# bryanlimy/tf2-cyclegan

Hardware: AMD Instinct MI355X
Metric: images/sec (whole node) horse2zebra 256×256 (higher is better)
Workload: dtype bf16; 1 GPU; model=cyclegan-resnet9-patchgan, global_batch=4, per_gpu_batch=4, image_size=256, parallelism=dp1

## Files before the change

### cyclegan_amd/ops/_hip/bind.cpp

```cpp
#include <torch/extension.h>

namespace cyg {
at::Tensor conv2d_fwd(at::Tensor, at::Tensor, c10::optional<at::Tensor>,
                      int64_t, int64_t, int64_t, int64_t, int64_t, bool,
                      int64_t, double);
at::Tensor convt2d_fwd(at::Tensor, at::Tensor, c10::optional<at::Tensor>,
                       int64_t, int64_t, int64_t, int64_t, int64_t, int64_t,
                       double);
std::vector<at::Tensor> conv2d_fwd_stats(at::Tensor, at::Tensor,
                                         c10::optional<at::Tensor>, int64_t,
                                         int64_t, int64_t, int64_t, int64_t,
                                         bool, int64_t, double);
std::vector<at::Tensor> convt2d_fwd_stats(at::Tensor, at::Tensor,
                                          c10::optional<at::Tensor>, int64_t,
                                          int64_t, int64_t, int64_t, int64_t,
                                          int64_t, double);
at::Tensor conv2d_dgrad(at::Tensor, at::Tensor, int64_t, int64_t, int64_t,
                        int64_t, int64_t, int64_t, int64_t, bool);
at::Tensor convt2d_dgrad(at::Tensor, at::Tensor, int64_t, int64_t, int64_t,
                         int64_t, int64_t);
at::Tensor conv2d_wgrad(at::Tensor, at::Tensor, int64_t, int64_t, int64_t,
                        int64_t, int64_t, bool);
at::Tensor mfma_probe(at::Tensor, at::Tensor);
at::Tensor mx_probe(at::Tensor, at::Tensor, int64_t, int64_t);
at::Tensor mx_probe16(at::Tensor, at::Tensor, int64_t, int64_t);
at::Tensor glds_probe(at::Tensor, at::Tensor);
at::Tensor tr_probe(int64_t);
at::Tensor quant_fp8(at::Tensor, at::Tensor);
at::Tensor quant_fp8_d(at::Tensor, at::Tensor, at::Tensor);
void amax_roll(at::Tensor, int64_t);
at::Tensor conv2d_fp8_fwd(at::Tensor, at::Tensor, at::Tensor,
                          c10::optional<at::Tensor>, c10::optional<at::Tensor>,
                          int64_t, int64_t, int64_t, int64_t, int64_t, bool, int64_t, double);
std::vector<at::Tensor> conv2d_fp8_fwd_stats(
    at::Tensor, at::Tensor, at::Tensor, c10::optional<at::Tensor>,
    c10::optional<at::Tensor>, int64_t, int64_t, int64_t, int64_t, int64_t,
    bool, int64_t, double);
std::vector<at::Tensor> instnorm_fwd(at::Tensor, at::Tensor, at::Tensor,
                                     double, int64_t, double,
                                     c10::optional<at::Tensor>,
                                     c10::optional<at::Tensor>,
                                     c10::optional<at::Tensor>, int64_t);
std::vector<at::Tensor> instnorm_fwd_q8(at::Tensor, at::Tensor, at::Tensor,
                                        double, int64_t, double,
                                        c10::optional<at::Tensor>,
                                        c10::optional<at::Tensor>,
                                        c10::optional<at::Tensor>, int64_t,
                                        at::Tensor, at::Tensor);
std::vector<at::Tensor> instnorm_bwd(at::Tensor, at::Tensor, at::Tensor,
                                     at::Tensor, at::Tensor,
                                     c10::optional<at::Tensor>, int64_t,
                                     double, c10::optional<at::Tensor>);
at::Tensor act_bwd(at::Tensor, at::Tensor, int64_t, double);
at::Tensor channel_sum(at::Tensor);
at::Tensor reflect_pad_fwd(at::Tensor, int64_t, int64_t, int64_t, int64_t);
at::Tensor reflect_pad_bwd(at::Tensor, int64_t, int64_t, int64_t, int64_t);
at::Tensor persample_loss_fwd(at::Tensor, at::Tensor, bool);
at::Tensor persample_loss_const_fwd(at::Tensor, double, bool);
std::vector<at::Tensor> persample_loss_bwd(at::Tensor, at::Tensor, at::Tensor,
                                           bool, bool, bool);
at::Tensor persample_loss_const_bwd(at::Tensor, double, at::Tensor, bool);
void adam_step_dev(at::Tensor, at::Tensor, at::Tensor, at::Tensor, at::Tensor,
                   double, double, double);
void shadow_gather(at::Tensor, at::Tensor, at::Tensor);
void adam_step(at::Tensor, at::Tensor, at::Tensor, at::Tensor, double, double,
               double, double, int64_t);
at::Tensor augment_batch(at::Tensor, at::Tensor, at::Tensor, int64_t, int64_t,
                         at::Tensor);
}

PYBIND11_MODULE(TORCH_EXTENSION_NAME, m) {
  m.def("conv2d_fwd", &cyg::conv2d_fwd);
  m.def("convt2d_fwd", &cyg::convt2d_fwd);
  m.def("conv2d_fwd_stats", &cyg::conv2d_fwd_stats);
  m.def("convt2d_fwd_stats", &cyg::convt2d_fwd_stats);
  m.def("conv2d_dgrad", &cyg::conv2d_dgrad);
  m.def("convt2d_dgrad", &cyg::convt2d_dgrad);
  m.def("conv2d_wgrad", &cyg::conv2d_wgrad);
  m.def("mfma_probe", &cyg::mfma_probe);
  m.def("mx_probe", &cyg::mx_probe);
  m.def("mx_probe16", &cyg::mx_probe16);
  m.def("glds_probe", &cyg::glds_probe);
  m.def("tr_probe", &cyg::tr_probe);
  m.def("quant_fp8", &cyg::quant_fp8);
  m.def("quant_fp8_d", &cyg::quant_fp8_d);
  m.def("amax_roll", &cyg::amax_roll);
  m.def("conv2d_fp8_fwd", &cyg::conv2d_fp8_fwd);
  m.def("conv2d_fp8_fwd_stats", &cyg::conv2d_fp8_fwd_stats);
  m.def("instnorm_fwd", &cyg::instnorm_fwd, py::arg("x"), py::arg("gamma"),
        py::arg("beta"), py::arg("eps"), py::arg("act"), py::arg("slope"),
        py::arg("residual"), py::arg("psum") = py::none(),
        py::arg("psq") = py::none(), py::arg("nslabs") = 0);
  m.def("instnorm_fwd_q8", &cyg::instnorm_fwd_q8, py::arg("x"),
        py::arg("gamma"), py::arg("beta"), py::arg("eps"), py::arg("act"),
        py::arg("slope"), py::arg("residual"), py::arg("psum"),
        py::arg("psq"), py::arg("nslabs"), py::arg("amax_prev"),
        py::arg("amax_cur"));
  m.def("instnorm_bwd", &cyg::instnorm_bwd, py::arg("dy"), py::arg("x"),
        py::arg("gamma"), py::arg("mean"), py::arg("rstd"), py::arg("yact"),
        py::arg("act"), py::arg("slope"), py::arg("beta") = py::none());
  m.def("act_bwd", &cyg::act_bwd);
  m.def("channel_sum", &cyg::channel_sum);
  m.def("reflect_pad_fwd", &cyg::reflect_pad_fwd);
  m.def("reflect_pad_bwd", &cyg::reflect_pad_bwd);
  m.def("persample_loss_fwd", &cyg::persample_loss_fwd);
  m.def("persample_loss_const_fwd", &cyg::persample_loss_const_fwd);
  m.def("persample_loss_bwd", &cyg::persample_loss_bwd);
  m.def("persample_loss_const_bwd", &cyg::persample_loss_const_bwd);
  m.def("adam_step", &cyg::adam_step);
  m.def("adam_step_dev", &cyg::adam_step_dev);
  m.def("shadow_gather", &cyg::shadow_gather);
  m.def("augment_batch", &cyg::augment_batch);
}
```

### cyclegan_amd/ops/_hip/conv.hip

```cpp

#include <torch/extension.h>
#include <ATen/cuda/CUDAContext.h>

#include "common.h"

namespace cyg {

constexpr int BM = 128, BN = 64, BK = 64;
constexpr int NTHREADS = 256;
constexpr int LDK = BK + 8;

struct ConvParams {
  const short* __restrict__ x;
  const short* __restrict__ w;
  const short* __restrict__ bias;
  short* __restrict__ y;
  int B, H, W, Cin, OH, OW, Cout, KH, KW;
  int stride, pt, pl;
  int reflect;
  int act;  float slope;
  const float* dq;
  const float* dqb;
  long M, KTOT;
  int mtiles, ntiles;
// ... 1397 lines not shown
  if (k >= KTOT || n >= Cout) return;
  long stride = (long)ktiles * ntiles * wbn * WG_BK;
  long off = (((long)kt * ntiles + nt) * wbn + nl) * WG_BK + kl;
  float s0 = 0, s1 = 0, s2 = 0, s3 = 0;
  int sl = 0;
  for (; sl + 4 <= slices; sl += 4) {
    s0 += ws[off + (sl + 0) * stride];
    s1 += ws[off + (sl + 1) * stride];
    s2 += ws[off + (sl + 2) * stride];
    s3 += ws[off + (sl + 3) * stride];
  }
  for (; sl < slices; ++sl) s0 += ws[off + sl * stride];
  dw[(long)n * KTOT + k] = (s0 + s1) + (s2 + s3);
}

__global__ void reflect_fold_kernel(const short* __restrict__ dxp,
                                    short* __restrict__ dx,
                                    int B, int H, int W, int C,
                                    int pt, int pb, int pl, int pr) {
  long idx = (long)blockIdx.x * blockDim.x + threadIdx.x;
  int gpr = C / 8;
  long total = (long)B * H * W * gpr;
  if (idx >= total) return;
  int g = (int)(idx % gpr);
  long t = idx / gpr;
  int j = (int)(t % W);
  t /= W;
  int i = (int)(t % H);
  int b = (int)(t / H);
  int HP = H + pt + pb, WP = W + pl + pr;
// ... 421 lines not shown
                              hipStream_t stream) {
  constexpr size_t SMB = sizeof(WgSmemT<WBN>);
  if constexpr (WBN == 128) {
    static bool init = []() {
      hipFuncSetAttribute((const void*)(wgrad_glds_kernel<128>),
                          hipFuncAttributeMaxDynamicSharedMemorySize,
                          (int)SMB);
      return true;
    }();
    (void)init;
  }
  hipLaunchKernelGGL((wgrad_glds_kernel<WBN>), grid, dim3(NW * 64), SMB,
                     stream, p);
}

at::Tensor conv2d_wgrad(at::Tensor x, at::Tensor dy, int64_t KH, int64_t KW,
                        int64_t stride, int64_t pt, int64_t pl, bool reflect) {
  TORCH_CHECK(x.is_cuda() && dy.is_cuda() && x.is_contiguous() && dy.is_contiguous());
  TORCH_CHECK(x.scalar_type() == at::kBFloat16 && dy.scalar_type() == at::kBFloat16);
  TORCH_CHECK(dy.size(0) == x.size(0));
  WgradParams p{};
  p.x = (const short*)x.const_data_ptr();
  p.dy = (const short*)dy.const_data_ptr();
  p.B = x.size(0); p.H = x.size(1); p.W = x.size(2); p.Cin = x.size(3);
  p.OH = dy.size(1); p.OW = dy.size(2); p.Cout = dy.size(3);
  p.KH = KH; p.KW = KW; p.stride = stride; p.pt = pt; p.pl = pl;
  p.reflect = reflect ? 1 : 0;
  p.M = (long)p.B * p.OH * p.OW;
  p.KTOT = (long)KH * KW * p.Cin;
  const bool glds_ok = (p.Cin % 8) == 0 && (p.Cout % 8) == 0 &&
                       (long)p.B * p.H * p.W * p.Cin * 2 < (1L << 31) &&
                       p.M * p.Cout * 2 < (1L << 31);
  const int wbn = glds_ok ? conv_ntile(p.Cout) : WG_BN;
  p.ktiles = cdiv(p.KTOT, WG_BK);
  p.ntiles = cdiv(p.Cout, wbn);
  const WgSplit split = wgrad_split(p.M, p.ktiles, p.ntiles);
  p.slices = split.slices;
  p.mchunks_per_slice = split.mchunks_per_slice;
  dim3 grid((long)p.ktiles * p.ntiles * p.slices);
  auto stream = at::cuda::getCurrentCUDAStream();
  if (!glds_ok) {
    auto dw = at::zeros({p.Cout, (long)KH, (long)KW, p.Cin},
                        x.options().dtype(at::kFloat));
    p.dw = (float*)dw.mutable_data_ptr();
    hipLaunchKernelGGL(wgrad_kernel, grid, dim3(NTHREADS), 0, stream, p);
    return dw;
  }
  auto dw = at::empty({p.Cout, (long)KH, (long)KW, p.Cin},
                      x.options().dtype(at::kFloat));
  p.dw = (float*)dw.mutable_data_ptr();
  auto ws = at::empty({(long)p.slices * p.ktiles * p.ntiles * wbn * WG_BK},
                      x.options().dtype(at::kFloat));
  p.ws = (float*)ws.mutable_data_ptr();
  switch (wbn) {
    case 16: launch_wgrad_glds<16>(p, grid, stream); break;
    case 128: launch_wgrad_glds<128>(p, grid, stream); break;
    default: launch_wgrad_glds<64>(p, grid, stream);
  }
  long total = (long)p.ktiles * WG_BK * p.ntiles * wbn;
  hipLaunchKernelGGL(wgrad_reduce_kernel, dim3(cdiv(total, 256)),
                     dim3(256), 0, stream,
                     (const float*)ws.const_data_ptr(), p.dw, p.KTOT,
                     p.Cout, p.ktiles, p.ntiles, p.slices, wbn);
  return dw;
}

at::Tensor quant_fp8(at::Tensor x, at::Tensor scale) {
  TORCH_CHECK(x.is_cuda() && x.scalar_type() == at::kBFloat16 && x.is_contiguous());
  TORCH_CHECK(scale.scalar_type() == at::kFloat);
  auto y = at::empty_like(x, x.options().dtype(at::kByte));
  long n = x.numel();
  long blocks = (n / 8 + 255) / 256 + 1;
  hipLaunchKernelGGL(quant_fp8_kernel, dim3((unsigned)blocks), dim3(256), 0,
                     at::cuda::getCurrentCUDAStream(),
                     (const short*)x.const_data_ptr(),
                     (const float*)scale.const_data_ptr(),
                     (unsigned char*)y.mutable_data_ptr(), n);
  return y;
}
// ... 91 lines not shown
```

### cyclegan_amd/ops/_hip/norm_elem.hip

```cpp

#include <torch/extension.h>
#include <ATen/cuda/CUDAContext.h>

#include "common.h"

namespace cyg {

constexpr int NT = 256;

static inline int cdiv64(long a, long b) { return (int)((a + b - 1) / b); }

__global__ __launch_bounds__(NT) void in_reduce_kernel(
    const short* __restrict__ x, float* __restrict__ psum,
    float* __restrict__ psq, int B, long HW, int C, int S) {
  int b = blockIdx.x / S;
  int sl = blockIdx.x % S;
  long rows = (HW + S - 1) / S;
  long r0 = sl * rows, r1 = min(r0 + rows, HW);
  const int gpr = C / 8;
  const int tid = threadIdx.x;
  const short* xb = x + (long)b * HW * C;

  int g = tid % gpr;
  int rstep = NT / gpr;
// ... 175 lines not shown
constexpr int MASK_NONE = 0, MASK_YACT = 1, MASK_X = 2;
DEV float actbw(float d, float yy, int act, float slope) {
  if (act == ACT_RELU) return yy > 0.f ? d : 0.f;
  if (act == ACT_LRELU) return yy > 0.f ? d : d * slope;
  if (act == ACT_TANH) return d * (1.f - yy * yy);
  return d;
}

template <int MM>
__global__ __launch_bounds__(NT) void in_bwd_reduce_kernel(
    const short* __restrict__ dy, const short* __restrict__ x,
    const short* __restrict__ yact, const float* __restrict__ gamma,
    const float* __restrict__ beta, const float* __restrict__ mean,
    const float* __restrict__ rstd,
    float* __restrict__ p1, float* __restrict__ p2, int B, long HW, int C,
    int S, int act, float slope, float* __restrict__ dgb) {
  int b = blockIdx.x / S;
  int sl = blockIdx.x % S;
  if (blockIdx.x == 0)
    for (int i = threadIdx.x; i < 2 * C; i += NT) dgb[i] = 0.f;
  long rows = (HW + S - 1) / S;
  long r0 = sl * rows, r1 = min(r0 + rows, HW);
  const int gpr = C / 8;
  const int tid = threadIdx.x;
  const long base = (long)b * HW * C;

  int g = tid % gpr;
  int rstep = NT / gpr;
  int rof = tid / gpr;
  float a1[8] = {}, a2[8] = {};
  float mv[8], rv[8], gv[8] = {}, bv[8] = {};
  #pragma unroll
  for (int j = 0; j < 8; ++j) {
    mv[j] = mean[(long)b * C + g * 8 + j];
    rv[j] = rstd[(long)b * C + g * 8 + j];
// ... 153 lines not shown
        float xh = (xf - smean[c]) * rs;
        float d = b2f(dv[j]);
        if (MM == MASK_YACT) d = actbw(d, b2f(yv[j]), act, slope);
        if (MM == MASK_X)
          d = actbw(d, in_affine(xf, smean[c], rs, gamma[c], beta[c]), act,
                    slope);
        out[j] = f2b(gamma[c] * rs * (d - sm1[c] - xh * sm2[c]));
      }
      *(v8s*)(dx + off) = out;
    }
  }
}

__global__ __launch_bounds__(NT) void channel_sum_kernel(
    const short* __restrict__ x, float* __restrict__ out, long rows, int C,
    int S) {
  int sl = blockIdx.x;
  long per = (rows + S - 1) / S;
  long r0 = sl * per, r1 = min(r0 + per, rows);
  const int gpr = C / 8;
  const int tid = threadIdx.x;
  int g = tid % gpr;
  int rstep = NT / gpr;
  int rof = tid / gpr;
  float a[8] = {};
  for (long r = r0 + rof; r < r1; r += rstep) {
    v8s v = *(const v8s*)(x + r * C + g * 8);
    #pragma unroll
    for (int j = 0; j < 8; ++j) a[j] += b2f(v[j]);
  }
  __shared__ float red[NT * 17];
  #pragma unroll
  for (int j = 0; j < 8; ++j) red[tid * 17 + j] = a[j];
  __syncthreads();
  for (int c = tid; c < C; c += NT) {
    int g2 = c / 8, j = c % 8;
    float t = 0;
    for (int k = 0; k < rstep; ++k) t += red[(g2 + k * gpr) * 17 + j];
    atomicAdd(&out[c], t);
  }
}

__global__ void act_bwd_kernel(const short* __restrict__ dy,
                               const short* __restrict__ y,
                               short* __restrict__ out, long n, int act,
                               float slope) {
  long i = ((long)blockIdx.x * blockDim.x + threadIdx.x) * 8;
  if (i >= n) return;
  if (i + 8 <= n) {
    v8s dv = *(const v8s*)(dy + i);
// ... 305 lines not shown
      hipLaunchKernelGGL(kern<MASK_X>, grid, dim3(NT), 0, stream,           \
                         __VA_ARGS__);                                      \
    else if ((mm) == MASK_YACT)                                             \
      hipLaunchKernelGGL(kern<MASK_YACT>, grid, dim3(NT), 0, stream,        \
                         __VA_ARGS__);                                      \
    else                                                                    \
      hipLaunchKernelGGL(kern<MASK_NONE>, grid, dim3(NT), 0, stream,        \
                         __VA_ARGS__);                                      \
  } while (0)

std::vector<at::Tensor> instnorm_bwd(at::Tensor dy, at::Tensor x,
                                     at::Tensor gamma, at::Tensor mean,
                                     at::Tensor rstd,
                                     c10::optional<at::Tensor> yact,
                                     int64_t act, double slope,
                                     c10::optional<at::Tensor> beta) {
  TORCH_CHECK(dy.is_cuda() && dy.scalar_type() == at::kBFloat16 &&
              dy.is_contiguous() && x.is_contiguous());
  TORCH_CHECK(act == ACT_NONE || yact.has_value() ||
              ((act == ACT_RELU || act == ACT_LRELU) && beta.has_value()),
              "instnorm_bwd: act ", act, " needs yact (or beta for relu/lrelu)");
  TORCH_CHECK(!beta.has_value() ||
              (beta->scalar_type() == at::kFloat && beta->numel() == x.size(3)),
              "instnorm_bwd: beta must be fp32 [C]");
  const float* betap =
      beta.has_value() ? (const float*)beta->const_data_ptr() : nullptr;
  const int mm = act == ACT_NONE ? MASK_NONE
                                 : (yact.has_value() ? MASK_YACT : MASK_X);
  int B = x.size(0), C = x.size(3);
  long HW = (long)x.size(1) * x.size(2);
  TORCH_CHECK(C % 8 == 0 && (C / 8) <= 256 && 256 % std::min(C / 8, 256) == 0,
              "instnorm_bwd: unsupported channel count ", C);
  auto stream = at::cuda::getCurrentCUDAStream();
  auto fopt = x.options().dtype(at::kFloat);
  int S = slices_for(HW, B);
  auto dx = at::empty_like(x);
  auto dgb = at::empty({2, C}, fopt);
  auto dbeta = dgb[0];
  auto dgamma = dgb[1];
  const short* yp = yact.has_value()
                        ? (const short*)yact->const_data_ptr() : nullptr;

  auto p1 = at::empty({S, B, C}, fopt);
  auto p2 = at::empty({S, B, C}, fopt);
  LAUNCH_MM(in_bwd_reduce_kernel, mm, dim3(B * S), stream,
                     (const short*)dy.const_data_ptr(),
                     (const short*)x.const_data_ptr(), yp,
                     (const float*)gamma.const_data_ptr(), betap,
                     (const float*)mean.const_data_ptr(),
                     (const float*)rstd.const_data_ptr(),
                     (float*)p1.mutable_data_ptr(),
                     (float*)p2.mutable_data_ptr(), B, HW, C, S, (int)act,
                     (float)slope, (float*)dgb.mutable_data_ptr());
  LAUNCH_MM(in_bwd_dx_kernel, mm, dim3(B * S), stream,
                     (const short*)dy.const_data_ptr(),
                     (const short*)x.const_data_ptr(), yp,
                     (const float*)gamma.const_data_ptr(), betap,
                     (const float*)mean.const_data_ptr(),
                     (const float*)rstd.const_data_ptr(),
                     (const float*)p1.const_data_ptr(),
                     (const float*)p2.const_data_ptr(),
                     (short*)dx.mutable_data_ptr(),
                     (float*)dbeta.mutable_data_ptr(),
                     (float*)dgamma.mutable_data_ptr(), B, HW, C, S,
                     (int)act, (float)slope);
  return {dx, dgamma, dbeta};
}

at::Tensor channel_sum(at::Tensor x) {
  TORCH_CHECK(x.is_cuda() && x.scalar_type() == at::kBFloat16 && x.is_contiguous());
  int C = x.size(-1);
  long rows = x.numel() / C;
  TORCH_CHECK(C % 8 == 0 && (C / 8) <= NT && NT % (C / 8) == 0,
              "channel_sum: unsupported C ", C);
  auto out = at::empty({C}, x.options().dtype(at::kFloat));
  CHECK_HIP(hipMemsetAsync(out.mutable_data_ptr(), 0, C * sizeof(float),
                           at::cuda::getCurrentCUDAStream()));
  int S = (int)std::min<long>(512, std::max<long>(1, rows / 64));
  hipLaunchKernelGGL(channel_sum_kernel, dim3(S), dim3(NT), 0,
                     at::cuda::getCurrentCUDAStream(),
                     (const short*)x.const_data_ptr(),
                     (float*)out.mutable_data_ptr(), rows, C, S);
  return out;
}

at::Tensor act_bwd(at::Tensor dy, at::Tensor y, int64_t act, double slope) {
  TORCH_CHECK(dy.is_cuda() && dy.scalar_type() == at::kBFloat16);
  auto out = at::empty_like(dy);
  long n = dy.numel();
  long blocks = (n / 8 + 255) / 256 + 1;
  hipLaunchKernelGGL(act_bwd_kernel, dim3((unsigned)blocks), dim3(256), 0,
                     at::cuda::getCurrentCUDAStream(),
                     (const short*)dy.const_data_ptr(),
                     (const short*)y.const_data_ptr(),
                     (short*)out.mutable_data_ptr(), n, (int)act,
                     (float)slope);
  return out;
// ... 154 lines not shown
```

### cyclegan_amd/ops/conv.py

```python

from __future__ import annotations

import os
from typing import NamedTuple, Optional, Tuple

import torch
import torch.nn.functional as F

from . import backend
from .shadow import (compute_weight, compute_weight_t, compute_weight_p,
                     compute_weight_tp, compute_bias_p, compute_weight_packp,
                     compute_bias_packb, fp8_weight_shadow)

ACT_NONE, ACT_RELU, ACT_LRELU, ACT_TANH = 0, 1, 2, 3

_ACT = {None: ACT_NONE, "none": ACT_NONE, "relu": ACT_RELU, "lrelu": ACT_LRELU, "tanh": ACT_TANH}


def same_pads(in_h: int, in_w: int, kh: int, kw: int, stride: int) -> Tuple[int, int, int, int]:
    out_h = -(-in_h // stride)
    out_w = -(-in_w // stride)
    ph = max(0, (out_h - 1) * stride + kh - in_h)
    pw = max(0, (out_w - 1) * stride + kw - in_w)
    return ph // 2, ph - ph // 2, pw // 2, pw - pw // 2
# ... 65 lines not shown
    @staticmethod
    def forward(ctx, x, w, bias, stride, pads, reflect, act, slope):
        ext = backend.ext()
        cout = w.shape[0]
        xp = _pad_channels(x).contiguous()
        wc = compute_weight_p(w, x)
        bc = compute_bias_p(bias, x) if bias is not None else None
        slabs = ()
        if _want_stats(bias, act) and cout >= 8:
            y, *slabs = ext.conv2d_fwd_stats(xp, wc, bc, stride, *pads,
                                             reflect, act, slope)
        else:
            y = ext.conv2d_fwd(xp, wc, bc, stride, *pads, reflect, act, slope)
        if cout < 8:
            y = y[..., :cout].contiguous()
        ctx.save_for_backward(xp, w, y)
        ctx.conf = (stride, pads, reflect, act, slope, bias is not None,
                    x.shape[3])
        if slabs:
            ctx.set_materialize_grads(False)
            ctx.mark_non_differentiable(*slabs)
            return (y, *slabs)
        return y

    @staticmethod
    def backward(ctx, dy, *_):
        if dy is None:
            return (None,) * 8
        xp, w, y = ctx.saved_tensors
        stride, pads, reflect, act, slope, has_bias, cin = ctx.conf
        cout = w.shape[0]
        pt, pb, pl, pr = pads
        ext = backend.ext()
        dy = dy.contiguous()
        if act != ACT_NONE:
            dy = ext.act_bwd(dy, y, act, slope)
        dyp = _pad_channels(dy).contiguous()
        db = None
        if has_bias and ctx.needs_input_grad[2]:
            db = ext.channel_sum(dyp)[: dy.shape[-1]]
        dx = dw = None
        if ctx.needs_input_grad[0]:
            wt = compute_weight_tp(w, xp)
            dx = ext.conv2d_dgrad(dyp, wt, xp.shape[1], xp.shape[2], stride,
                                  pt, pb, pl, pr, reflect)
            if cin < 8:
                dx = dx[..., :cin].contiguous()
        if ctx.needs_input_grad[1]:
            dw = ext.conv2d_wgrad(xp, dyp, w.shape[1], w.shape[2], stride,
                                  pt, pl, reflect)
            if cout < 8 or cin < 8:
                dw = dw[:cout, :, :, :cin].contiguous()
            if dw.dtype != w.dtype:
                dw = dw.to(w.dtype)
        return dx, dw, db, None, None, None, None, None


def _head_packable(x, w, stride, pads, reflect) -> bool:
    import os
    if os.environ.get("CYG_NO_PACKHEAD") == "1":
        return False
    return (reflect and stride == 1 and pads == (3, 3, 3, 3)
            and w.shape[0] <= 8 and w.shape[1] == 7 and w.shape[2] == 7
            and w.shape[3] % 8 == 0 and w.shape[3] >= 8
            and x.shape[2] % 8 == 0 and x.shape[1] >= 7 and x.shape[2] >= 16)


def _fold_packed_dw(dwp: torch.Tensor, wshape) -> torch.Tensor:
    O, KH, KW, I = wshape
    d6 = dwp.view(8, 8, KH, 2, 8, I)
# ... 9 lines not shown
class _ConvHeadPackedFn(torch.autograd.Function):

    @staticmethod
    def forward(ctx, x, w, bias, act, slope):
        ext = backend.ext()
        B, H, W, Cin = x.shape
        cout = w.shape[0]
        wpk = compute_weight_packp(w, x)
        bpk = compute_bias_packb(bias, x) if bias is not None else None
        xp = ext.reflect_pad_fwd(x.contiguous(), 3, 3, 3, 5)
        xf = xp.view(B, H + 6, (W + 8) // 8, 8 * Cin)
        yp = ext.conv2d_fwd(xf, wpk, bpk, 1, 0, 0, 0, 0, False, act, slope)
        y = yp.view(B, H, W, 8)
        if cout < 8:
            y = y[..., :cout].contiguous()
        ctx.save_for_backward(xp, w, y)
        ctx.conf = (act, slope, bias is not None, cout, Cin, H, W)
        return y

    @staticmethod
    def backward(ctx, dy):
        xp, w, y = ctx.saved_tensors
        act, slope, has_bias, cout, Cin, H, W = ctx.conf
        ext = backend.ext()
        dy = dy.contiguous()
        if act != ACT_NONE:
            dy = ext.act_bwd(dy, y, act, slope)
        dyp = _pad_channels(dy).contiguous()
        db = None
        if has_bias and ctx.needs_input_grad[2]:
            db = ext.channel_sum(dyp)[: dy.shape[-1]]
        dx = dw = None
        B = dyp.shape[0]
        if ctx.needs_input_grad[0]:
            wt = compute_weight_tp(w, xp)
            dx = ext.conv2d_dgrad(dyp, wt, H, W, 1, 3, 3, 3, 3, True)
        if ctx.needs_input_grad[1]:
            xf = xp.view(B, H + 6, (W + 8) // 8, 8 * Cin)
            dy_pk = dyp.view(B, H, W // 8, 64)
            dwp = ext.conv2d_wgrad(xf, dy_pk, 7, 2, 1, 0, 0, False)
            dw = _fold_packed_dw(dwp, tuple(w.shape))
            if dw.dtype != w.dtype:
                dw = dw.to(w.dtype)
        return dx, dw, db, None, None


_FP8_MODE = False


def set_fp8_mode(on: bool):
    global _FP8_MODE
    _FP8_MODE = bool(on)


def fp8_mode() -> bool:
    return _FP8_MODE


# ... 53 lines not shown
        if fresh:
            prev.copy_(xp.detach().abs().amax().float().clamp(min=1e-12))
            twin = None
        xq = twin if twin is not None else ext.quant_fp8_d(xp, prev, cur)
        bc = compute_bias_p(bias, x) if bias is not None else None
        slabs = ()
        if (_want_stats(bias, act) and cout >= 8
                and not _knob_off("CYG_NO_FP8_STATS")):
            y, *slabs = ext.conv2d_fp8_fwd_stats(xq, wq, prev, sw, bc, stride,
                                                 *pads, reflect, act, slope)
        else:
            y = ext.conv2d_fp8_fwd(xq, wq, prev, sw, bc, stride, *pads,
                                   reflect, act, slope)
        if cout < 8:
            y = y[..., :cout].contiguous()
        ctx.save_for_backward(xp, w, y)
        ctx.conf = (stride, pads, reflect, act, slope, bias is not None,
                    x.shape[3])
        if slabs:
            ctx.set_materialize_grads(False)
            ctx.mark_non_differentiable(*slabs)
            return (y, *slabs)
        return y

    @staticmethod
    def backward(ctx, dy, *_):
        return _ConvFn.backward(ctx, dy) + (None,)


class _ConvTFn(torch.autograd.Function):
    @staticmethod
# ... 11 lines not shown
        ctx.save_for_backward(x, w, y)
        ctx.conf = (stride, pt, pl, act, slope, bias is not None)
        if slabs:
            ctx.set_materialize_grads(False)
            ctx.mark_non_differentiable(*slabs)
            return (y, *slabs)
        return y

    @staticmethod
    def backward(ctx, dy, *_):
        if dy is None:
            return (None,) * 10
        x, w, y = ctx.saved_tensors
        stride, pt, pl, act, slope, has_bias = ctx.conf
        ext = backend.ext()
        dy = dy.contiguous()
        if act != ACT_NONE:
            dy = ext.act_bwd(dy, y, act, slope)
        dx = dw = db = None
        if ctx.needs_input_grad[0]:
            wt = compute_weight_t(w, x)
            dx = ext.convt2d_dgrad(dy, wt, x.shape[1], x.shape[2], stride, pt, pl)
        if ctx.needs_input_grad[1]:
            dwc = ext.conv2d_wgrad(dy, x, w.shape[1], w.shape[2], stride,
                                   pt, pl, False)
            dw = dwc.permute(3, 1, 2, 0).contiguous()
            if dw.dtype != w.dtype:
                dw = dw.to(w.dtype)
        if has_bias and ctx.needs_input_grad[2]:
            db = dy.float().sum(dim=(0, 1, 2))
        return dx, dw, db, None, None, None, None, None, None, None


def conv2d(
    x: torch.Tensor,
    w: torch.Tensor,
    bias: Optional[torch.Tensor] = None,
    stride: int = 1,
    padding: str | Tuple[int, int, int, int] = "valid",
    pad_mode: str = "zeros",
    act: Optional[str] = None,
    slope: float = 0.2,
) -> torch.Tensor:
# ... 43 lines not shown
```

### cyclegan_amd/ops/norm.py

```python

from __future__ import annotations

import os
from typing import Optional

import torch

from . import backend
from . import conv as _conv
from .conv import (ACT_NONE, ACT_RELU, ACT_LRELU, FP8_TWIN_ATTR,
                   IN_SLABS_ATTR, _ACT, Fp8Consumer)

EPS_DEFAULT = 1e-3


def _in_ref(x, gamma, beta, eps, act, slope, residual):
    cdt = torch.float32 if x.dtype == torch.bfloat16 else x.dtype
    xf = x.to(cdt)
    mean = xf.mean(dim=(1, 2), keepdim=True)
    var = xf.var(dim=(1, 2), unbiased=False, keepdim=True)
    y = (xf - mean) * torch.rsqrt(var + eps)
    y = y * gamma.to(cdt) + beta.to(cdt)
    y = y.to(x.dtype)
    if residual is not None:
# ... 33 lines not shown
        ctx.conf = (eps, act, slope, residual is not None)
        if yq is not None:
            ctx.set_materialize_grads(False)
            ctx.mark_non_differentiable(yq)
            return y, yq
        return y

    @staticmethod
    def backward(ctx, dy, *_):
        if dy is None:
            return (None,) * 11
        x, gamma, mean, rstd, y, betaf = ctx.saved_tensors
        eps, act, slope, has_res = ctx.conf
        ext = backend.ext()
        dy = dy.contiguous()
        if has_res and act != ACT_NONE:
            dy = ext.act_bwd(dy, y, act, slope)
            dres = dy
            dx, dgamma, dbeta = ext.instnorm_bwd(dy, x, gamma.float(), mean,
                                                 rstd, None, ACT_NONE, 0.0)
        else:
            dres = dy if has_res else None
            yact = y if (act != ACT_NONE and not _mask_from_x(act)) else None
            dx, dgamma, dbeta = ext.instnorm_bwd(
                dy, x, gamma.float(), mean, rstd, yact, act, slope, betaf)
        return (dx, dgamma.to(gamma.dtype), dbeta, None, None, None, dres,
                None, None, None, None)


def _slabs_for(x: torch.Tensor):
    st = getattr(x, IN_SLABS_ATTR, None)
    if st is None or x.dim() != 4:
        return None, None
    psum, psq = st
    want = (x.shape[0], x.shape[3])
    if (psum.dim() != 3 or tuple(psum.shape[1:]) != want
            or psq.shape != psum.shape or psum.device != x.device):
        return None, None
    return psum, psq


# ... 32 lines not shown
```

### cyclegan_amd/parallel/flat.py

```python

from __future__ import annotations

from typing import List

import torch


class FlatParamGroup:
    def __init__(self, module: torch.nn.Module):
        params: List[torch.nn.Parameter] = [p for p in module.parameters() if p.requires_grad]
        assert all(p.dtype == torch.float32 for p in params), "master params must be fp32"
        n = sum(p.numel() for p in params)
        dev = params[0].device
        self.flat_param = torch.empty(n, dtype=torch.float32, device=dev)
        self.flat_grad = torch.zeros(n, dtype=torch.float32, device=dev)
        self.params = params
        self._offsets = []
        off = 0
        with torch.no_grad():
            for p in params:
                k = p.numel()
                self.flat_param[off:off + k].copy_(p.detach().reshape(-1))
                p.data = self.flat_param[off:off + k].view(p.shape)
                self._offsets.append((off, k))
                off += k
        self.attach_grads()

    def attach_grads(self):
        for p, (off, k) in zip(self.params, self._offsets):
            p.grad = self.flat_grad[off:off + k].view(p.shape)

    def bump_versions(self):
        for p in self.params:
            torch.autograd.graph.increment_version(p)

    def set_grads(self, grads):
        torch._foreach_copy_(
            [p.grad for p in self.params],
            [g.reshape(p.shape) for p, g in zip(self.params, grads)])

    def zero_grad(self):
        self.flat_grad.zero_()
        self.attach_grads()

    def check_views(self) -> bool:
        pp = self.flat_param.data_ptr()
        gp = self.flat_grad.data_ptr()
        ok = True
        for p in self.params:
            ok &= p.data.data_ptr() >= pp and p.data.data_ptr() < pp + self.flat_param.numel() * 4
            ok &= p.grad is not None and gp <= p.grad.data_ptr() < gp + self.flat_grad.numel() * 4
        return ok
```

### cyclegan_amd/trainer.py

```python

from __future__ import annotations

import os
from typing import Dict, Optional

import torch

from .models import Generator, Discriminator
from .ops import MAE, MSE, MSE_const, backend
from .ops.adam import FusedAdam
from .parallel import DistContext, GradSync, FlatParamGroup


class CycleGAN:
    LAMBDA_CYCLE = 10.0
    LAMBDA_IDENTITY = 0.5 * 10.0

    def __init__(self, args, ctx: DistContext):
        self.ctx = ctx
        self.device = ctx.device
        self.global_batch_size = args.global_batch_size
        self.compute_dtype = getattr(args, "compute_dtype", None) or (
            torch.bfloat16 if self.device.type == "cuda" else torch.float32)
        self._fp8 = bool(getattr(args, "fp8", False))
# ... 109 lines not shown
            "loss_F/loss": F_loss, "loss_F/cycle": F_cycle_loss,
            "loss_F/identity": F_identity_loss,
            "loss_F/total": F_loss + F_cycle_loss + F_identity_loss,
            "loss_X/loss": self.discriminator_loss(self.X(x),
                                                   discriminate_fake_x),
            "loss_Y/loss": self.discriminator_loss(self.Y(y),
                                                   discriminate_fake_y),
        }

    _GROUP_LOSS = (("G", "loss_G/total"), ("F", "loss_F/total"),
                   ("X", "loss_X/loss"), ("Y", "loss_Y/loss"))

    def _grads_for(self, losses: Dict[str, torch.Tensor], name: str,
                   retain: bool):
        key = dict(self._GROUP_LOSS)[name]
        self.groups[name].set_grads(
            torch.autograd.grad(losses[key], self.groups[name].params,
                                retain_graph=retain))

    def _optimize(self):
        for opt in self.optimizers.values():
            opt.step()
        for g in self.groups.values():
            g.bump_versions()
        self._refresh_shadows()
        if getattr(self, "_fp8", False):
            from .ops import fp8_state
            fp8_state.roll()

    def train_step(self, x, y) -> Dict[str, torch.Tensor]:
        x, y = self._cast(x), self._cast(y)
        if x.shape[0] == 0:
            return self._empty_train_step()
# ... 237 lines not shown
```

Baseline: 340.2 images/s.

## Write weight and norm gradients directly into flat gradient buffers via grad sink

Adds a grad-sink mechanism so conv wgrad, transposed-conv wgrad, packed-7x7 fold, instnorm bwd and bias channel_sum write (or accumulate) fp32 gradients straight into the flat parameter gradient views, instead of returning temporaries that are permuted, cast and then copied with foreach_copy. It also skips weight-gradient computation for frozen leaf parameters that are not in the current group, so each autograd.grad call only computes wgrad for its own group. This cuts extra kernels, allocations and copies in backward. The cost is global state coupling autograd functions to the trainer, and accumulate paths that rely on touched flags.

```diff
diff --git a/cyclegan_amd/ops/_hip/bind.cpp b/cyclegan_amd/ops/_hip/bind.cpp
--- a/cyclegan_amd/ops/_hip/bind.cpp
+++ b/cyclegan_amd/ops/_hip/bind.cpp
@@ -21,6 +21,9 @@
                          int64_t, int64_t);
 at::Tensor conv2d_wgrad(at::Tensor, at::Tensor, int64_t, int64_t, int64_t,
                         int64_t, int64_t, bool);
+void conv2d_wgrad_into(at::Tensor, at::Tensor, int64_t, int64_t, int64_t,
+                       int64_t, int64_t, bool, at::Tensor, bool, bool);
+void fold_packed_dw_into(at::Tensor, at::Tensor, bool);
 at::Tensor mfma_probe(at::Tensor, at::Tensor);
 at::Tensor mx_probe(at::Tensor, at::Tensor, int64_t, int64_t);
 at::Tensor mx_probe16(at::Tensor, at::Tensor, int64_t, int64_t);
@@ -50,9 +53,11 @@
 std::vector<at::Tensor> instnorm_bwd(at::Tensor, at::Tensor, at::Tensor,
                                      at::Tensor, at::Tensor,
                                      c10::optional<at::Tensor>, int64_t,
-                                     double, c10::optional<at::Tensor>);
+                                     double, c10::optional<at::Tensor>,
+                                     c10::optional<at::Tensor>,
+                                     c10::optional<at::Tensor>, bool);
 at::Tensor act_bwd(at::Tensor, at::Tensor, int64_t, double);
-at::Tensor channel_sum(at::Tensor);
+at::Tensor channel_sum(at::Tensor, c10::optional<at::Tensor>, bool);
 at::Tensor reflect_pad_fwd(at::Tensor, int64_t, int64_t, int64_t, int64_t);
 at::Tensor reflect_pad_bwd(at::Tensor, int64_t, int64_t, int64_t, int64_t);
 at::Tensor persample_loss_fwd(at::Tensor, at::Tensor, bool);
@@ -77,6 +82,12 @@
   m.def("conv2d_dgrad", &cyg::conv2d_dgrad);
   m.def("convt2d_dgrad", &cyg::convt2d_dgrad);
   m.def("conv2d_wgrad", &cyg::conv2d_wgrad);
+  m.def("conv2d_wgrad_into", &cyg::conv2d_wgrad_into, py::arg("x"),
+        py::arg("dy"), py::arg("kh"), py::arg("kw"), py::arg("stride"),
+        py::arg("pt"), py::arg("pl"), py::arg("reflect"), py::arg("out"),
+        py::arg("accumulate"), py::arg("transpose_oi") = false);
+  m.def("fold_packed_dw_into", &cyg::fold_packed_dw_into, py::arg("dwp"),
+        py::arg("out"), py::arg("accumulate"));
   m.def("mfma_probe", &cyg::mfma_probe);
   m.def("mx_probe", &cyg::mx_probe);
   m.def("mx_probe16", &cyg::mx_probe16);
@@ -98,9 +109,12 @@
         py::arg("amax_cur"));
   m.def("instnorm_bwd", &cyg::instnorm_bwd, py::arg("dy"), py::arg("x"),
         py::arg("gamma"), py::arg("mean"), py::arg("rstd"), py::arg("yact"),
-        py::arg("act"), py::arg("slope"), py::arg("beta") = py::none());
+        py::arg("act"), py::arg("slope"), py::arg("beta") = py::none(),
+        py::arg("dgamma_out") = py::none(), py::arg("dbeta_out") = py::none(),
+        py::arg("accumulate") = false);
   m.def("act_bwd", &cyg::act_bwd);
-  m.def("channel_sum", &cyg::channel_sum);
+  m.def("channel_sum", &cyg::channel_sum, py::arg("x"),
+        py::arg("out") = py::none(), py::arg("accumulate") = false);
   m.def("reflect_pad_fwd", &cyg::reflect_pad_fwd);
   m.def("reflect_pad_bwd", &cyg::reflect_pad_bwd);
   m.def("persample_loss_fwd", &cyg::persample_loss_fwd);
diff --git a/cyclegan_amd/ops/_hip/conv.hip b/cyclegan_amd/ops/_hip/conv.hip
--- a/cyclegan_amd/ops/_hip/conv.hip
+++ b/cyclegan_amd/ops/_hip/conv.hip
@@ -1435,6 +1435,66 @@
   dw[(long)n * KTOT + k] = (s0 + s1) + (s2 + s3);
 }
 
+__global__ void wgrad_reduce_into_kernel(const float* __restrict__ ws,
+                                         float* __restrict__ out, long KTOT,
+                                         int Cout, int ktiles, int ntiles,
+                                         int slices, int wbn, int cin_g,
+                                         int taps, int co_true, int ci_true,
+                                         int tr, int accum) {
+  long idx = (long)blockIdx.x * blockDim.x + threadIdx.x;
+  long total = (long)ktiles * WG_BK * ntiles * wbn;
+  if (idx >= total) return;
+  int kl = (int)(idx % WG_BK);
+  long t = idx / WG_BK;
+  int kt = (int)(t % ktiles);
+  t /= ktiles;
+  int nl = (int)(t % wbn);
+  int nt = (int)(t / wbn);
+  long k = (long)kt * WG_BK + kl;
+  int n = nt * wbn + nl;
+  if (k >= KTOT || n >= Cout) return;
+  int tap = (int)(k / cin_g);
+  int ci = (int)(k - (long)tap * cin_g);
+  if (n >= co_true || ci >= ci_true) return;
+  long stride = (long)ktiles * ntiles * wbn * WG_BK;
+  long off = (((long)kt * ntiles + nt) * wbn + nl) * WG_BK + kl;
+  float s0 = 0, s1 = 0, s2 = 0, s3 = 0;
+  int sl = 0;
+  for (; sl + 4 <= slices; sl += 4) {
+    s0 += ws[off + (sl + 0) * stride];
+    s1 += ws[off + (sl + 1) * stride];
+    s2 += ws[off + (sl + 2) * stride];
+    s3 += ws[off + (sl + 3) * stride];
+  }
+  for (; sl < slices; ++sl) s0 += ws[off + sl * stride];
+  float s = (s0 + s1) + (s2 + s3);
+  long o = tr ? ((long)ci * taps + tap) * co_true + n
+              : ((long)n * taps + tap) * ci_true + ci;
+  out[o] = accum ? out[o] + s : s;
+}
+
+__global__ void fold_packed_dw_kernel(const float* __restrict__ dwp,
+                                      float* __restrict__ out, int O, int KH,
+                                      int KW, int I, int accum) {
+  long idx = (long)blockIdx.x * blockDim.x + threadIdx.x;
+  long total = (long)O * KH * KW * I;
+  if (idx >= total) return;
+  int ci = (int)(idx % I);
+  long t = idx / I;
+  int tx = (int)(t % KW);
+  t /= KW;
+  int ty = (int)(t % KH);
+  int co = (int)(t / KH);
+  float s = 0.f;
+  #pragma unroll
+  for (int d = 0; d < 8; ++d) {
+    int a = tx + d;
+    s += dwp[((((long)(d * 8 + co) * KH + ty) * 2 + (a >> 3)) * 8 + (a & 7)) *
+                 I + ci];
+  }
+  out[idx] = accum ? out[idx] + s : s;
+}
+
 __global__ void reflect_fold_kernel(const short* __restrict__ dxp,
                                     short* __restrict__ dx,
                                     int B, int H, int W, int C,
@@ -1886,8 +1946,10 @@
                      stream, p);
 }
 
-at::Tensor conv2d_wgrad(at::Tensor x, at::Tensor dy, int64_t KH, int64_t KW,
-                        int64_t stride, int64_t pt, int64_t pl, bool reflect) {
+static at::Tensor wgrad_impl(at::Tensor x, at::Tensor dy, int64_t KH,
+                             int64_t KW, int64_t stride, int64_t pt,
+                             int64_t pl, bool reflect, const at::Tensor* into,
+                             bool accumulate, bool transpose_oi) {
   TORCH_CHECK(x.is_cuda() && dy.is_cuda() && x.is_contiguous() && dy.is_contiguous());
   TORCH_CHECK(x.scalar_type() == at::kBFloat16 && dy.scalar_type() == at::kBFloat16);
   TORCH_CHECK(dy.size(0) == x.size(0));
@@ -1916,11 +1978,18 @@
                         x.options().dtype(at::kFloat));
     p.dw = (float*)dw.mutable_data_ptr();
     hipLaunchKernelGGL(wgrad_kernel, grid, dim3(NTHREADS), 0, stream, p);
-    return dw;
-  }
-  auto dw = at::empty({p.Cout, (long)KH, (long)KW, p.Cin},
-                      x.options().dtype(at::kFloat));
-  p.dw = (float*)dw.mutable_data_ptr();
+    if (!into) return dw;
+    auto v = transpose_oi ? dw.permute({3, 1, 2, 0}) : dw;
+    v = v.narrow(0, 0, into->size(0)).narrow(3, 0, into->size(3));
+    if (accumulate) into->add_(v); else into->copy_(v);
+    return *into;
+  }
+  at::Tensor dw;
+  if (!into) {
+    dw = at::empty({p.Cout, (long)KH, (long)KW, p.Cin},
+                   x.options().dtype(at::kFloat));
+    p.dw = (float*)dw.mutable_data_ptr();
+  }
   auto ws = at::empty({(long)p.slices * p.ktiles * p.ntiles * wbn * WG_BK},
                       x.options().dtype(at::kFloat));
   p.ws = (float*)ws.mutable_data_ptr();
@@ -1930,11 +1999,67 @@
     default: launch_wgrad_glds<64>(p, grid, stream);
   }
   long total = (long)p.ktiles * WG_BK * p.ntiles * wbn;
-  hipLaunchKernelGGL(wgrad_reduce_kernel, dim3(cdiv(total, 256)),
+  if (!into) {
+    hipLaunchKernelGGL(wgrad_reduce_kernel, dim3(cdiv(total, 256)),
+                       dim3(256), 0, stream,
+                       (const float*)ws.const_data_ptr(), p.dw, p.KTOT,
+                       p.Cout, p.ktiles, p.ntiles, p.slices, wbn);
+    return dw;
+  }
+  const int co_true = (int)into->size(transpose_oi ? 3 : 0);
+  const int ci_true = (int)into->size(transpose_oi ? 0 : 3);
+  hipLaunchKernelGGL(wgrad_reduce_into_kernel, dim3(cdiv(total, 256)),
                      dim3(256), 0, stream,
-                     (const float*)ws.const_data_ptr(), p.dw, p.KTOT,
-                     p.Cout, p.ktiles, p.ntiles, p.slices, wbn);
-  return dw;
+                     (const float*)ws.const_data_ptr(),
+                     (float*)into->mutable_data_ptr(), p.KTOT, p.Cout,
+                     p.ktiles, p.ntiles, p.slices, wbn, p.Cin, (int)(KH * KW),
+                     co_true, ci_true, transpose_oi ? 1 : 0,
+                     accumulate ? 1 : 0);
+  return *into;
+}
+
+at::Tensor conv2d_wgrad(at::Tensor x, at::Tensor dy, int64_t KH, int64_t KW,
+                        int64_t stride, int64_t pt, int64_t pl, bool reflect) {
+  return wgrad_impl(x, dy, KH, KW, stride, pt, pl, reflect, nullptr, false,
+                    false);
+}
+
+static void check_grad_dest(const at::Tensor& out, const char* who) {
+  TORCH_CHECK(out.is_cuda() && out.scalar_type() == at::kFloat &&
+                  out.is_contiguous(),
+              who, ": out must be a contiguous fp32 device tensor");
+}
+
+void conv2d_wgrad_into(at::Tensor x, at::Tensor dy, int64_t KH, int64_t KW,
+                       int64_t stride, int64_t pt, int64_t pl, bool reflect,
+                       at::Tensor out, bool accumulate, bool transpose_oi) {
+  check_grad_dest(out, "conv2d_wgrad_into");
+  TORCH_CHECK(out.dim() == 4 && out.size(1) == KH && out.size(2) == KW,
+              "conv2d_wgrad_into: out must be [O,KH,KW,I]");
+  const int64_t co = out.size(transpose_oi ? 3 : 0);
+  const int64_t ci = out.size(transpose_oi ? 0 : 3);
+  TORCH_CHECK(co >= 1 && co <= dy.size(3) && ci >= 1 && ci <= x.size(3),
+              "conv2d_wgrad_into: out channels exceed the GEMM's");
+  wgrad_impl(x, dy, KH, KW, stride, pt, pl, reflect, &out, accumulate,
+             transpose_oi);
+}
+
+void fold_packed_dw_into(at::Tensor dwp, at::Tensor out, bool accumulate) {
+  check_grad_dest(out, "fold_packed_dw_into");
+  TORCH_CHECK(dwp.is_cuda() && dwp.scalar_type() == at::kFloat &&
+              dwp.is_contiguous() && dwp.dim() == 4 && out.dim() == 4);
+  const int64_t O = out.size(0), KH = out.size(1), KW = out.size(2),
+                I = out.size(3);
+  TORCH_CHECK(O >= 1 && O <= 8 && KW >= 1 && KW <= 9 && dwp.size(0) == 64 &&
+                  dwp.size(1) == KH && dwp.size(2) == 2 &&
+                  dwp.size(3) == 8 * I,
+              "fold_packed_dw_into: shape mismatch");
+  long total = out.numel();
+  hipLaunchKernelGGL(fold_packed_dw_kernel, dim3(cdiv(total, 256)), dim3(256),
+                     0, at::cuda::getCurrentCUDAStream(),
+                     (const float*)dwp.const_data_ptr(),
+                     (float*)out.mutable_data_ptr(), (int)O, (int)KH, (int)KW,
+                     (int)I, accumulate ? 1 : 0);
 }
 
 at::Tensor quant_fp8(at::Tensor x, at::Tensor scale) {
diff --git a/cyclegan_amd/ops/_hip/norm_elem.hip b/cyclegan_amd/ops/_hip/norm_elem.hip
--- a/cyclegan_amd/ops/_hip/norm_elem.hip
+++ b/cyclegan_amd/ops/_hip/norm_elem.hip
@@ -213,11 +213,15 @@
     const float* __restrict__ beta, const float* __restrict__ mean,
     const float* __restrict__ rstd,
     float* __restrict__ p1, float* __restrict__ p2, int B, long HW, int C,
-    int S, int act, float slope, float* __restrict__ dgb) {
+    int S, int act, float slope, float* __restrict__ zbeta,
+    float* __restrict__ zgamma) {
   int b = blockIdx.x / S;
   int sl = blockIdx.x % S;
-  if (blockIdx.x == 0)
-    for (int i = threadIdx.x; i < 2 * C; i += NT) dgb[i] = 0.f;
+  if (blockIdx.x == 0 && zbeta != nullptr)
+    for (int i = threadIdx.x; i < C; i += NT) {
+      zbeta[i] = 0.f;
+      zgamma[i] = 0.f;
+    }
   long rows = (HW + S - 1) / S;
   long r0 = sl * rows, r1 = min(r0 + rows, HW);
   const int gpr = C / 8;
@@ -401,7 +405,7 @@
 
 __global__ __launch_bounds__(NT) void channel_sum_kernel(
     const short* __restrict__ x, float* __restrict__ out, long rows, int C,
-    int S) {
+    int S, int nout) {
   int sl = blockIdx.x;
   long per = (rows + S - 1) / S;
   long r0 = sl * per, r1 = min(r0 + per, rows);
@@ -420,7 +424,7 @@
   #pragma unroll
   for (int j = 0; j < 8; ++j) red[tid * 17 + j] = a[j];
   __syncthreads();
-  for (int c = tid; c < C; c += NT) {
+  for (int c = tid; c < nout; c += NT) {
     int g2 = c / 8, j = c % 8;
     float t = 0;
     for (int k = 0; k < rstep; ++k) t += red[(g2 + k * gpr) * 17 + j];
@@ -756,9 +760,21 @@
                                      at::Tensor rstd,
                                      c10::optional<at::Tensor> yact,
                                      int64_t act, double slope,
-                                     c10::optional<at::Tensor> beta) {
+                                     c10::optional<at::Tensor> beta,
+                                     c10::optional<at::Tensor> dgamma_out,
+                                     c10::optional<at::Tensor> dbeta_out,
+                                     bool accumulate) {
   TORCH_CHECK(dy.is_cuda() && dy.scalar_type() == at::kBFloat16 &&
               dy.is_contiguous() && x.is_contiguous());
+  TORCH_CHECK(dgamma_out.has_value() == dbeta_out.has_value(),
+              "instnorm_bwd: pass both destinations or neither");
+  TORCH_CHECK(!accumulate || dgamma_out.has_value(),
+              "instnorm_bwd: accumulate needs destinations");
+  if (dgamma_out.has_value())
+    for (const at::Tensor* t : {&*dgamma_out, &*dbeta_out})
+      TORCH_CHECK(t->is_cuda() && t->scalar_type() == at::kFloat &&
+                      t->is_contiguous() && t->numel() == x.size(3),
+                  "instnorm_bwd: destinations must be contiguous fp32 [C]");
   TORCH_CHECK(act == ACT_NONE || yact.has_value() ||
               ((act == ACT_RELU || act == ACT_LRELU) && beta.has_value()),
               "instnorm_bwd: act ", act, " needs yact (or beta for relu/lrelu)");
@@ -777,9 +793,17 @@
   auto fopt = x.options().dtype(at::kFloat);
   int S = slices_for(HW, B);
   auto dx = at::empty_like(x);
-  auto dgb = at::empty({2, C}, fopt);
-  auto dbeta = dgb[0];
-  auto dgamma = dgb[1];
+  at::Tensor dbeta, dgamma;
+  if (dgamma_out.has_value()) {
+    dbeta = *dbeta_out;
+    dgamma = *dgamma_out;
+  } else {
+    auto dgb = at::empty({2, C}, fopt);
+    dbeta = dgb[0];
+    dgamma = dgb[1];
+  }
+  float* zb = accumulate ? nullptr : (float*)dbeta.mutable_data_ptr();
+  float* zg = accumulate ? nullptr : (float*)dgamma.mutable_data_ptr();
   const short* yp = yact.has_value()
                         ? (const short*)yact->const_data_ptr() : nullptr;
 
@@ -793,7 +817,7 @@
                      (const float*)rstd.const_data_ptr(),
                      (float*)p1.mutable_data_ptr(),
                      (float*)p2.mutable_data_ptr(), B, HW, C, S, (int)act,
-                     (float)slope, (float*)dgb.mutable_data_ptr());
+                     (float)slope, zb, zg);
   LAUNCH_MM(in_bwd_dx_kernel, mm, dim3(B * S), stream,
                      (const short*)dy.const_data_ptr(),
                      (const short*)x.const_data_ptr(), yp,
@@ -809,20 +833,34 @@
   return {dx, dgamma, dbeta};
 }
 
-at::Tensor channel_sum(at::Tensor x) {
+at::Tensor channel_sum(at::Tensor x, c10::optional<at::Tensor> dest,
+                       bool accumulate) {
   TORCH_CHECK(x.is_cuda() && x.scalar_type() == at::kBFloat16 && x.is_contiguous());
   int C = x.size(-1);
   long rows = x.numel() / C;
   TORCH_CHECK(C % 8 == 0 && (C / 8) <= NT && NT % (C / 8) == 0,
               "channel_sum: unsupported C ", C);
-  auto out = at::empty({C}, x.options().dtype(at::kFloat));
-  CHECK_HIP(hipMemsetAsync(out.mutable_data_ptr(), 0, C * sizeof(float),
-                           at::cuda::getCurrentCUDAStream()));
+  TORCH_CHECK(!accumulate || dest.has_value(),
+              "channel_sum: accumulate needs a destination");
+  at::Tensor out;
+  if (dest.has_value()) {
+    out = *dest;
+    TORCH_CHECK(out.is_cuda() && out.scalar_type() == at::kFloat &&
+                    out.is_contiguous() && out.numel() >= 1 &&
+                    out.numel() <= C,
+                "channel_sum: out must be contiguous fp32 of <= C elements");
+  } else {
+    out = at::empty({C}, x.options().dtype(at::kFloat));
+  }
+  const int nout = (int)out.numel();
+  if (!accumulate)
+    CHECK_HIP(hipMemsetAsync(out.mutable_data_ptr(), 0, nout * sizeof(float),
+                             at::cuda::getCurrentCUDAStream()));
   int S = (int)std::min<long>(512, std::max<long>(1, rows / 64));
   hipLaunchKernelGGL(channel_sum_kernel, dim3(S), dim3(NT), 0,
                      at::cuda::getCurrentCUDAStream(),
                      (const short*)x.const_data_ptr(),
-                     (float*)out.mutable_data_ptr(), rows, C, S);
+                     (float*)out.mutable_data_ptr(), rows, C, S, nout);
   return out;
 }
 
diff --git a/cyclegan_amd/ops/conv.py b/cyclegan_amd/ops/conv.py
--- a/cyclegan_amd/ops/conv.py
+++ b/cyclegan_amd/ops/conv.py
@@ -7,7 +7,7 @@
 import torch
 import torch.nn.functional as F
 
-from . import backend
+from . import backend, grad_sink
 from .shadow import (compute_weight, compute_weight_t, compute_weight_p,
                      compute_weight_tp, compute_bias_p, compute_weight_packp,
                      compute_bias_packb, fp8_weight_shadow)
@@ -103,7 +103,7 @@
             y = ext.conv2d_fwd(xp, wc, bc, stride, *pads, reflect, act, slope)
         if cout < 8:
             y = y[..., :cout].contiguous()
-        ctx.save_for_backward(xp, w, y)
+        ctx.save_for_backward(xp, w, y, bias)
         ctx.conf = (stride, pads, reflect, act, slope, bias is not None,
                     x.shape[3])
         if slabs:
@@ -116,18 +116,19 @@
     def backward(ctx, dy, *_):
         if dy is None:
             return (None,) * 8
-        xp, w, y = ctx.saved_tensors
+        xp, w, y, bias = ctx.saved_tensors
         stride, pads, reflect, act, slope, has_bias, cin = ctx.conf
         cout = w.shape[0]
         pt, pb, pl, pr = pads
         ext = backend.ext()
+        sink = grad_sink.current()
         dy = dy.contiguous()
         if act != ACT_NONE:
             dy = ext.act_bwd(dy, y, act, slope)
         dyp = _pad_channels(dy).contiguous()
         db = None
         if has_bias and ctx.needs_input_grad[2]:
-            db = ext.channel_sum(dyp)[: dy.shape[-1]]
+            db = _bias_grad(ext, sink, bias, dyp, dy.shape[-1])
         dx = dw = None
         if ctx.needs_input_grad[0]:
             wt = compute_weight_tp(w, xp)
@@ -135,14 +136,27 @@
                                   pt, pb, pl, pr, reflect)
             if cin < 8:
                 dx = dx[..., :cin].contiguous()
-        if ctx.needs_input_grad[1]:
-            dw = ext.conv2d_wgrad(xp, dyp, w.shape[1], w.shape[2], stride,
-                                  pt, pl, reflect)
-            if cout < 8 or cin < 8:
-                dw = dw[:cout, :, :, :cin].contiguous()
-            if dw.dtype != w.dtype:
-                dw = dw.to(w.dtype)
+        if ctx.needs_input_grad[1] and not grad_sink.frozen(sink, w):
+            if sink is not None and sink.has(w):
+                out, acc = sink.take(w)
+                ext.conv2d_wgrad_into(xp, dyp, w.shape[1], w.shape[2], stride,
+                                      pt, pl, reflect, out, acc, False)
+            else:
+                dw = ext.conv2d_wgrad(xp, dyp, w.shape[1], w.shape[2], stride,
+                                      pt, pl, reflect)
+                if cout < 8 or cin < 8:
+                    dw = dw[:cout, :, :, :cin].contiguous()
         return dx, dw, db, None, None, None, None, None
+
+
+def _bias_grad(ext, sink, bias, dyp, n):
+    if grad_sink.frozen(sink, bias):
+        return None
+    if sink is not None and sink.has(bias):
+        out, acc = sink.take(bias)
+        ext.channel_sum(dyp, out, acc)
+        return None
+    return ext.channel_sum(dyp)[:n]
 
 
 def _head_packable(x, w, stride, pads, reflect) -> bool:
@@ -182,34 +196,37 @@
         y = yp.view(B, H, W, 8)
         if cout < 8:
             y = y[..., :cout].contiguous()
-        ctx.save_for_backward(xp, w, y)
+        ctx.save_for_backward(xp, w, y, bias)
         ctx.conf = (act, slope, bias is not None, cout, Cin, H, W)
         return y
 
     @staticmethod
     def backward(ctx, dy):
-        xp, w, y = ctx.saved_tensors
+        xp, w, y, bias = ctx.saved_tensors
         act, slope, has_bias, cout, Cin, H, W = ctx.conf
         ext = backend.ext()
+        sink = grad_sink.current()
         dy = dy.contiguous()
         if act != ACT_NONE:
             dy = ext.act_bwd(dy, y, act, slope)
         dyp = _pad_channels(dy).contiguous()
         db = None
         if has_bias and ctx.needs_input_grad[2]:
-            db = ext.channel_sum(dyp)[: dy.shape[-1]]
+            db = _bias_grad(ext, sink, bias, dyp, dy.shape[-1])
         dx = dw = None
         B = dyp.shape[0]
         if ctx.needs_input_grad[0]:
             wt = compute_weight_tp(w, xp)
             dx = ext.conv2d_dgrad(dyp, wt, H, W, 1, 3, 3, 3, 3, True)
-        if ctx.needs_input_grad[1]:
+        if ctx.needs_input_grad[1] and not grad_sink.frozen(sink, w):
             xf = xp.view(B, H + 6, (W + 8) // 8, 8 * Cin)
             dy_pk = dyp.view(B, H, W // 8, 64)
             dwp = ext.conv2d_wgrad(xf, dy_pk, 7, 2, 1, 0, 0, False)
-            dw = _fold_packed_dw(dwp, tuple(w.shape))
-            if dw.dtype != w.dtype:
-                dw = dw.to(w.dtype)
+            if sink is not None and sink.has(w):
+                out, acc = sink.take(w)
+                ext.fold_packed_dw_into(dwp, out, acc)
+            else:
+                dw = _fold_packed_dw(dwp, tuple(w.shape))
         return dx, dw, db, None, None
 
 
@@ -293,7 +310,7 @@
                                    reflect, act, slope)
         if cout < 8:
             y = y[..., :cout].contiguous()
-        ctx.save_for_backward(xp, w, y)
+        ctx.save_for_backward(xp, w, y, bias)
         ctx.conf = (stride, pads, reflect, act, slope, bias is not None,
                     x.shape[3])
         if slabs:
@@ -335,6 +352,7 @@
         x, w, y = ctx.saved_tensors
         stride, pt, pl, act, slope, has_bias = ctx.conf
         ext = backend.ext()
+        sink = grad_sink.current()
         dy = dy.contiguous()
         if act != ACT_NONE:
             dy = ext.act_bwd(dy, y, act, slope)
@@ -342,12 +360,15 @@
         if ctx.needs_input_grad[0]:
             wt = compute_weight_t(w, x)
             dx = ext.convt2d_dgrad(dy, wt, x.shape[1], x.shape[2], stride, pt, pl)
-        if ctx.needs_input_grad[1]:
-            dwc = ext.conv2d_wgrad(dy, x, w.shape[1], w.shape[2], stride,
-                                   pt, pl, False)
-            dw = dwc.permute(3, 1, 2, 0).contiguous()
-            if dw.dtype != w.dtype:
-                dw = dw.to(w.dtype)
+        if ctx.needs_input_grad[1] and not grad_sink.frozen(sink, w):
+            if sink is not None and sink.has(w):
+                out, acc = sink.take(w)
+                ext.conv2d_wgrad_into(dy, x, w.shape[1], w.shape[2], stride,
+                                      pt, pl, False, out, acc, True)
+            else:
+                dwc = ext.conv2d_wgrad(dy, x, w.shape[1], w.shape[2], stride,
+                                       pt, pl, False)
+                dw = dwc.permute(3, 1, 2, 0).contiguous()
         if has_bias and ctx.needs_input_grad[2]:
             db = dy.float().sum(dim=(0, 1, 2))
         return dx, dw, db, None, None, None, None, None, None, None
diff --git a/cyclegan_amd/ops/grad_sink.py b/cyclegan_amd/ops/grad_sink.py
--- /dev/null
+++ b/cyclegan_amd/ops/grad_sink.py
@@ -0,0 +1,57 @@
+
+from __future__ import annotations
+
+import os
+from contextlib import contextmanager
+from typing import Dict, Iterable, Optional, Tuple
+
+import torch
+
+
+class GradSink:
+
+    def __init__(self, params: Iterable[torch.Tensor],
+                 views: Iterable[torch.Tensor]):
+        self._slots: Dict[int, list] = {}
+        for p, v in zip(params, views):
+            assert v.dtype == torch.float32 and v.is_contiguous()
+            assert v.shape == p.shape
+            self._slots[p.data_ptr()] = [v, False]
+
+    def has(self, p: torch.Tensor) -> bool:
+        return p.data_ptr() in self._slots
+
+    def take(self, p: torch.Tensor) -> Tuple[torch.Tensor, bool]:
+        slot = self._slots[p.data_ptr()]
+        view, touched = slot
+        slot[1] = True
+        return view, touched
+
+    def touched(self, p: torch.Tensor) -> bool:
+        slot = self._slots.get(p.data_ptr())
+        return slot is not None and slot[1]
+
+
+_ACTIVE: Optional[GradSink] = None
+
+
+def current() -> Optional[GradSink]:
+    return _ACTIVE
+
+
+def enabled() -> bool:
+    return os.environ.get("CYG_NO_GRAD_SINK") != "1"
+
+
+@contextmanager
+def active(sink: Optional[GradSink]):
+    global _ACTIVE
+    prev, _ACTIVE = _ACTIVE, sink
+    try:
+        yield sink
+    finally:
+        _ACTIVE = prev
+
+
+def frozen(sink: Optional[GradSink], p: torch.Tensor) -> bool:
+    return sink is not None and p.is_leaf and not sink.has(p)
diff --git a/cyclegan_amd/ops/norm.py b/cyclegan_amd/ops/norm.py
--- a/cyclegan_amd/ops/norm.py
+++ b/cyclegan_amd/ops/norm.py
@@ -6,7 +6,7 @@
 
 import torch
 
-from . import backend
+from . import backend, grad_sink
 from . import conv as _conv
 from .conv import (ACT_NONE, ACT_RELU, ACT_LRELU, FP8_TWIN_ATTR,
                    IN_SLABS_ATTR, _ACT, Fp8Consumer)
@@ -71,17 +71,28 @@
         eps, act, slope, has_res = ctx.conf
         ext = backend.ext()
         dy = dy.contiguous()
+        sink = grad_sink.current()
+        dest = (None, None, False)
+        if sink is not None and sink.has(gamma) and sink.has(betaf):
+            dg_out, acc = sink.take(gamma)
+            db_out, acc_b = sink.take(betaf)
+            assert acc == acc_b
+            dest = (dg_out, db_out, acc)
         if has_res and act != ACT_NONE:
             dy = ext.act_bwd(dy, y, act, slope)
             dres = dy
             dx, dgamma, dbeta = ext.instnorm_bwd(dy, x, gamma.float(), mean,
-                                                 rstd, None, ACT_NONE, 0.0)
+                                                 rstd, None, ACT_NONE, 0.0,
+                                                 None, *dest)
         else:
             dres = dy if has_res else None
             yact = y if (act != ACT_NONE and not _mask_from_x(act)) else None
             dx, dgamma, dbeta = ext.instnorm_bwd(
-                dy, x, gamma.float(), mean, rstd, yact, act, slope, betaf)
-        return (dx, dgamma.to(gamma.dtype), dbeta, None, None, None, dres,
+                dy, x, gamma.float(), mean, rstd, yact, act, slope, betaf,
+                *dest)
+        if dest[0] is not None:
+            dgamma = dbeta = None
+        return (dx, dgamma, dbeta, None, None, None, dres,
                 None, None, None, None)
 
 
diff --git a/cyclegan_amd/parallel/flat.py b/cyclegan_amd/parallel/flat.py
--- a/cyclegan_amd/parallel/flat.py
+++ b/cyclegan_amd/parallel/flat.py
@@ -34,10 +34,25 @@
         for p in self.params:
             torch.autograd.graph.increment_version(p)
 
-    def set_grads(self, grads):
-        torch._foreach_copy_(
-            [p.grad for p in self.params],
-            [g.reshape(p.shape) for p, g in zip(self.params, grads)])
+    def grad_sink(self):
+        from ..ops import grad_sink
+        if not (self.flat_grad.is_cuda and grad_sink.enabled()):
+            return None
+        return grad_sink.GradSink(self.params, [p.grad for p in self.params])
+
+    def set_grads(self, grads, sink=None):
+        dst, src = [], []
+        for p, g in zip(self.params, grads):
+            if g is None:
+                assert sink is not None and sink.touched(p), \
+                    "a parameter received no gradient"
+            elif sink is not None and sink.touched(p):
+                p.grad.add_(g.reshape(p.shape))
+            else:
+                dst.append(p.grad)
+                src.append(g.reshape(p.shape))
+        if dst:
+            torch._foreach_copy_(dst, src)
 
     def zero_grad(self):
         self.flat_grad.zero_()
diff --git a/cyclegan_amd/trainer.py b/cyclegan_amd/trainer.py
--- a/cyclegan_amd/trainer.py
+++ b/cyclegan_amd/trainer.py
@@ -7,7 +7,7 @@
 import torch
 
 from .models import Generator, Discriminator
-from .ops import MAE, MSE, MSE_const, backend
+from .ops import MAE, MSE, MSE_const, backend, grad_sink
 from .ops.adam import FusedAdam
 from .parallel import DistContext, GradSync, FlatParamGroup
 
@@ -147,9 +147,13 @@
     def _grads_for(self, losses: Dict[str, torch.Tensor], name: str,
                    retain: bool):
         key = dict(self._GROUP_LOSS)[name]
-        self.groups[name].set_grads(
-            torch.autograd.grad(losses[key], self.groups[name].params,
-                                retain_graph=retain))
+        group = self.groups[name]
+        sink = group.grad_sink()
+        with grad_sink.active(sink):
+            grads = torch.autograd.grad(losses[key], group.params,
+                                        retain_graph=retain,
+                                        allow_unused=sink is not None)
+        group.set_grads(grads, sink)
 
     def _optimize(self):
         for opt in self.optimizers.values():
```

Result: faster. 350.0 images/s, median of 6 (+2.9%).
